# iamarkaj/AwesomeSLAM

Hardware: AMD Instinct MI355X
Metric: EKF/UKF filter-steps/s @ N_landmarks (higher is better)
Workload: dtype f32

## Files before the change

awesomeslam_amd/csrc/aslam_core.hip:

```cpp
#include "../../include/aslam_core.h"
#include "../../include/aslam_scan.h"

#include <hip/hip_runtime.h>

#include <cmath>
#include <cstdio>
#include <cstring>
#include <cstdlib>
#include <algorithm>
#include <mutex>
#include <string>
#include <type_traits>
#include <vector>

#include "ekf_small.h"
#include "ekf_large.h"
#include "ekf_large_launch.h"
#include "scan_front.h"
#if ASLAM_HAVE_UKF
#include "ukf_small.h"
#include "ukf_large.h"
#include "ukf_large_launch.h"
#endif

// ... 103 lines not shown
template <typename F> int with_large_view(aslam_ctx *c, F &&f)
{
        return c->cfg.dtype == ASLAM_F32 ? f(c->lv32) : f(c->lv64);
}

int seed_pose_block(double *P, size_t B, size_t NP)
{
        std::vector<double> blk(3 * NP, 0.0);
        for (int i = 0; i < 3; ++i)
                blk[(size_t)i * NP + i] = (double)KP_ROBOT_POSE;
        for (size_t b = 0; b < B; ++b)
                HIP_TRY(hipMemcpy(P + b * NP * NP, blk.data(), sizeof(double) * blk.size(), hipMemcpyHostToDevice));
        return ASLAM_OK;
}

template <typename T> int init_P_large(aslam_ctx *c, LargeView<T> &lv)
{
        const size_t B = c->cfg.batch, NP = c->NP;
        HIP_TRY(hipMemset(lv.P, 0, sizeof(double) * B * NP * NP));
        HIP_TRY(hipMemset(lv.G, 0, sizeof(T) * B * NP * NP));
        HIP_TRY(hipMemset(lv.S, 0, sizeof(T) * B * NP * NP));
        if (lv.Vw)
                HIP_TRY(hipMemset(lv.Vw, 0, sizeof(T) * B * NP * NP));
        return seed_pose_block(lv.P, B, NP);
}

int init_state(aslam_ctx *c)
{
        const int B = c->cfg.batch, NP = c->NP;
        DevView &d = c->dv;
        HIP_TRY(hipMemset(d.X, 0, sizeof(double) * B * NP));
        HIP_TRY(hipMemset(d.Z, 0, sizeof(double) * B * NP));
        if (!c->large)
                HIP_TRY(hipMemset(d.P, 0, sizeof(double) * (size_t)B * NP * NP));
        HIP_TRY(hipMemset(d.status, 0, sizeof(uint32_t) * B));
        HIP_TRY(hipMemset(d.sens_n, 0, sizeof(int) * B));
        HIP_TRY(hipMemset(d.wait_n, 0, sizeof(int) * B));
        std::vector<int> n(B, 3), fl(B, FLAG_INIT_X | FLAG_INIT_Z);
        std::vector<double> A(2 * (size_t)B, 0.0);
        for (int b = 0; b < B; ++b)
                A[2 * b] = 1.0;
        HIP_TRY(hipMemcpy(d.n, n.data(), sizeof(int) * B, hipMemcpyHostToDevice));
        HIP_TRY(hipMemcpy(d.flags, fl.data(), sizeof(int) * B, hipMemcpyHostToDevice));
        HIP_TRY(hipMemcpy(d.A, A.data(), sizeof(double) * 2 * B, hipMemcpyHostToDevice));
        if (c->large)
                return with_large_view(c, [&](auto &lv) { return init_P_large(c, lv); });
// ... 80 lines not shown

template <typename T> int alloc_large(aslam_ctx *c, LargeView<T> &lv)
{
        const size_t B = (size_t)c->cfg.batch, NP = (size_t)c->NP;
        const LargePlan plan = large_plan(sizeof(T) == 4, c->NP, c->cfg.batch, c->cfg.batch, c->lh.knobs);
        int rc = ASLAM_OK;
        auto A_ = [&](int r) {
                if (rc == ASLAM_OK)
                        rc = r;
        };
        lv.NP = c->NP;
        lv.xrows = c->cfg.filter == ASLAM_UKF ? 2 : 1;
        A_(dev_alloc(c, &lv.P, B * NP * NP, c->owned));
        c->largeP = lv.P;
        A_(dev_alloc(c, &lv.G, B * NP * NP, c->owned));
        A_(dev_alloc(c, &lv.S, B * NP * NP, c->owned));
        A_(dev_alloc(c, &lv.Hc, B * (NP / 2) * 4, c->owned));
        A_(dev_alloc(c, &lv.Y, B * NP, c->owned));
        A_(dev_alloc(c, &lv.Linv, B * LARGE_NB_MAX * LB * LB, c->owned));
        if (plan.need_Lpl)
                A_(dev_alloc(c, &lv.Lpl, B * LPlanes::per_filter((int)NP), c->owned));
        if (plan.need_Vw)
                A_(dev_alloc(c, &lv.Vw, B * NP * NP, c->owned));
        return rc;
}

#if ASLAM_HAVE_UKF
int ukf_large_alloc(aslam_ctx *c)
{
        const size_t B = (size_t)c->cfg.batch, NP = (size_t)c->NP;
        const size_t MP = 2 * NP + 16;
        UkfLargeView &u = c->ukfl;
        u.MP = (int)MP;
        int rc = dev_alloc(c, &u.D, B * NP * MP, c->owned);
        if (rc == ASLAM_OK)
                rc = dev_alloc(c, &u.DZ, B * NP * MP, c->owned);
        if (rc == ASLAM_OK)
                rc = dev_alloc(c, &u.XP, B * 3 * MP, c->owned);
        if (rc == ASLAM_OK)
                rc = dev_alloc(c, &u.Xbar, B * NP, c->owned);
        if (rc == ASLAM_OK)
                rc = dev_alloc(c, &u.sc, B * 8, c->owned);
        return rc;
}
#endif
}
// ... 691 lines not shown
                *stream_groups = c->large ? c->lh.last_groups : 0;
        if (chol_resident)
                *chol_resident = c->large && c->lh.last_plan.chain == LargeChain::F32_RESIDENT;
        if (launches_per_callback)
                *launches_per_callback = c->large ? c->lh.last_plan.launches : 1;
        return ASLAM_OK;
}

int aslam_kernel_info(aslam_ctx *c, char *name, int name_cap, int *grid, int *block, int *lds_bytes)
{
        if (!c)
                return fail(ASLAM_ERR_ARG, "null context");
        char buf[192];
        size_t lds = 0;
        if (c->large)
        {
                const LargePlan plan = large_plan(c->cfg.dtype == ASLAM_F32, c->NP, c->cfg.batch, c->cfg.batch, c->lh.knobs);
#if ASLAM_HAVE_UKF
                if (c->cfg.filter == ASLAM_UKF)
                        std::snprintf(buf, sizeof(buf), "ukf_large_wabt + large_update_panel<double> + large_syrk<double> (%d-launch chain per callback, 1 stream)",
                                      ukf_large_plan(c->NP).launches);
                else
#endif
                if (plan.chain == LargeChain::F32_RESIDENT)
                        std::snprintf(buf, sizeof(buf), "%s + %s + large_syrk_bf16x3 (%d-launch chain per callback, %d stream groups)",
                                      plan.chol16 ? "large_chol_bf16" : "large_chol_resident", plan.trsm16 ? "large_trsm_bf16" : "large_trsm_pipe<17>",
                                      plan.launches, c->lh.knobs.groups);
                else if (plan.chain == LargeChain::F32_RIGHT)
                        std::snprintf(buf, sizeof(buf), "large_right_step + large_syrk_bf16x3 (%d-launch chain per callback: one right-looking launch per block column)", plan.launches);
                else if (plan.chain == LargeChain::F32_LEFT)
                        std::snprintf(buf, sizeof(buf), "large_trsm_pipe<17> + large_syrk_bf16x3 (%d-launch chain per callback: multi-workgroup Cholesky)", plan.launches);
                else
                        std::snprintf(buf, sizeof(buf), "large_update_panel<double> (%d-launch chain per callback, %d stream groups)", plan.launches, c->lh.knobs.groups);
                lds = LargeLds::bytes(c->NP);
        }
        else if (c->cfg.filter == ASLAM_EKF)
        {
                std::snprintf(buf, sizeof(buf), "ekf_small_kernel<%d,0>", c->NT);
                lds = with_NT(c->NT, [](auto nt) -> size_t { return SmallLayout<decltype(nt)::value>::total; });
        }
#if ASLAM_HAVE_UKF
        else
        {
                std::snprintf(buf, sizeof(buf), "ukf_small_kernel<%d,0>", c->NT);
                lds = with_NT(c->NT, [](auto nt) -> size_t { return UkfLayout<decltype(nt)::value>::total; });
        }
#endif
// ... 16 lines not shown
```

awesomeslam_amd/csrc/ekf_large.h:

```cpp
#pragma once

#include <type_traits>

#include "small_common.h"

namespace aslam
{
constexpr int LB = 64;
constexpr int LARGE_OBS_CAP = 1024;
constexpr int LARGE_WAIT_CAP = 2048;
constexpr int LARGE_NP_MAX = 1088;
constexpr int LARGE_NB_MAX = LARGE_NP_MAX / LB;

template <typename T> struct LargeView
{
        int NP;
        double *P;
        T *G;
        T *S;
        double *Hc;
        double *Y;
        T *Linv;
        T *Vw;
        unsigned short *Lpl;
        int xrows;
};

typedef float f4 __attribute__((ext_vector_type(4)));
template <typename T> struct Mfma;
template <> struct Mfma<double>
{
        typedef d4 acc_t;
        static __device__ __forceinline__ acc_t zero()
        {
                return (acc_t){0.0, 0.0, 0.0, 0.0};
        }
        static __device__ __forceinline__ acc_t mma(double a, double b, acc_t c)
        {
                return __builtin_amdgcn_mfma_f64_16x16x4f64(a, b, c, 0, 0, 0);
        }
        static __device__ __forceinline__ int row(int lane, int r)
        {
                return (lane >> 4) + 4 * r;
        }
};
template <> struct Mfma<float>
{
        typedef f4 acc_t;
// ... 25 lines not shown
                const bf2 mm = __builtin_convertvector(r1, bf2);
                const f2 r2 = r1 - __builtin_convertvector(mm, f2);
                const bf2 ll = __builtin_convertvector(r2, bf2);
                h[e] = __builtin_bit_cast(unsigned, hh), m[e] = __builtin_bit_cast(unsigned, mm), l[e] = __builtin_bit_cast(unsigned, ll);
        }
}

struct LPlanes
{
        unsigned short *base;
        __host__ __device__ static size_t per_filter(int NP) { return (size_t)3 * NP * NP; }
        __host__ __device__ unsigned short *Lq(int b, int NP) const { return base + (size_t)b * per_filter(NP); }
        __host__ __device__ unsigned short *block(int b, int NP, int k, int j) const { return Lq(b, NP) + (size_t)(64 * k) * NP + 64 * j; }
};
__host__ __device__ __forceinline__ int lplane_pos(int c)
{
        return 32 * (c >> 5) + 8 * ((c >> 2) & 3) + 4 * ((c >> 4) & 1) + (c & 3);
}

__host__ __device__ __forceinline__ int large_blocks(int n, int xrows = 1)
{
        return (n + xrows + LB - 1) / LB;
}

struct LargeLds
{
        static __host__ __device__ size_t bytes(int NP)
        {
                size_t o = 0;
                o += 8 * (size_t)NP * 2;
                o += 4 * (size_t)LARGE_OBS_CAP * 6;
                o += 4 * (size_t)LARGE_WAIT_CAP * 5;
                o += 4 * (size_t)(NP / 2);
                o += 4 * (size_t)LARGE_OBS_CAP * 4 * 2;
                o += 4 * (size_t)NP;
                o = (o + 15) & ~(size_t)15;
                return o + sizeof(SmallShared);
        }
        static __device__ __forceinline__ SmallLds carve(unsigned char *smem, int NP)
        {
                SmallLds L;
                unsigned char *p = smem;
                L.Lt = nullptr;
                L.Dinv = nullptr;
                L.sY = nullptr;
                L.sU = nullptr;
// ... 810 lines not shown
                        }
                }
}

#ifndef ASLAM_XU_ROWS
#define ASLAM_XU_ROWS 8
#endif
constexpr int XU_ROWS = ASLAM_XU_ROWS;
template <int DIAG = 0, int PL = 0>
__global__ __launch_bounds__(256, 3) void large_syrk_bf16x3(DevView d, LargeView<float> lv, LPlanes vpl, int nfilters, const int *skipped)
{
        constexpr int TB = 128, KC = 32;
        constexpr int LDB = KC;
        typedef __bf16 bf8 __attribute__((ext_vector_type(8)));
        typedef unsigned u4 __attribute__((ext_vector_type(4)));
        typedef unsigned u2 __attribute__((ext_vector_type(2)));
        __shared__ __attribute__((aligned(16))) unsigned short As[3][TB * LDB];
        __shared__ __attribute__((aligned(16))) unsigned short Bs[3][TB * LDB];
        const int ntile = (lv.NP + TB - 1) / TB, nlow = ntile * (ntile + 1) / 2;
        const int slot = blockIdx.x >> 3;
        const int b = (slot / nlow) * 8 + (blockIdx.x & 7);
        if (b >= nfilters || skipped[b])
                return;
        const int n = d.n[b], NP = lv.NP;
        const int na = large_blocks(n) * LB;
        const int tl = slot % nlow;
        int rt = (int)((sqrtf(8.0f * (float)tl + 1.0f) - 1.0f) * 0.5f);
        while ((rt + 1) * (rt + 2) / 2 <= tl)
                ++rt;
        while (rt * (rt + 1) / 2 > tl)
                --rt;
        const int jt = tl - rt * (rt + 1) / 2;
        if (rt * TB >= n)
                return;
        const int tid = threadIdx.x, wave = tid >> 6, lane = tid & 63, li = lane & 15, lg = lane >> 4;
        const int wr = (wave >> 1) * 64, wc = (wave & 1) * 64;
        const float *G = lv.G + (size_t)b * NP * NP;
        double *P = lv.P + (size_t)b * NP * NP;
        constexpr int LPR = KC / 4, RPP = 256 / LPR, NPASS = TB / RPP;
        const int lrow = tid / LPR, lc0 = (tid % LPR) * 4;
        const float *Ap[NPASS], *Bp[NPASS];
#pragma unroll
        for (int q = 0; q < NPASS; ++q)
        {
                Ap[q] = G + (size_t)min(rt * TB + lrow + RPP * q, na - 1) * NP + lc0;
                Bp[q] = G + (size_t)min(jt * TB + lrow + RPP * q, na - 1) * NP + lc0;
        }
        f4 acc[4][4];
#pragma unroll
        for (int u = 0; u < 4; ++u)
#pragma unroll
                for (int v = 0; v < 4; ++v)
                        acc[u][v] = (f4){0.f, 0.f, 0.f, 0.f};
        f4 ta[NPASS], tb[NPASS];
        auto fetch = [&](int kc) {
                if constexpr (PL)
                        return;
#pragma unroll
                for (int q = 0; q < NPASS; ++q)
                {
                        ta[q] = *reinterpret_cast<const f4 *>(Ap[q] + kc);
                        tb[q] = *reinterpret_cast<const f4 *>(Bp[q] + kc);
                }
        };
        typedef __attribute__((address_space(3))) unsigned short lds_us;
        const __amdgpu_buffer_rsrc_t vrs = __builtin_amdgcn_make_buffer_rsrc(PL ? (void *)vpl.Lq(b, NP) : (void *)nullptr, 0, (int)(LPlanes::per_filter(NP) * 2), 0x00020000);
        const unsigned dma_vo = (unsigned)(((lane >> 2) * NP) * 2 + (((lane & 3) ^ (lane >> 4)) * 16));
        const unsigned ldsA = (unsigned)__builtin_amdgcn_readfirstlane((int)((unsigned)(uintptr_t)(lds_us *)&As[0][0] + (unsigned)wave * 2048u));
        const unsigned ldsB = (unsigned)__builtin_amdgcn_readfirstlane((int)((unsigned)(uintptr_t)(lds_us *)&Bs[0][0] + (unsigned)wave * 2048u));
        auto dma_slab = [&](int kc) {
                const unsigned plane_b = (unsigned)(NP * NP * 2);
                const unsigned soA = (unsigned)__builtin_amdgcn_readfirstlane(((rt * TB + 32 * wave) * NP + kc) * 2);
                const unsigned soB = (unsigned)__builtin_amdgcn_readfirstlane(((jt * TB + 32 * wave) * NP + kc) * 2);
                const unsigned r16 = (unsigned)(16 * NP * 2);
#pragma unroll
                for (int p = 0; p < 3; ++p)
#pragma unroll
                        for (int jj = 0; jj < 2; ++jj)
                        {
                                asm volatile("s_add_u32 m0, %0, %1\n\ts_nop 0\n\tbuffer_load_dwordx4 %2, %3, %4 offen lds"
                                             :
                                             : "s"(ldsA), "n"(p * TB * LDB * 2 + jj * 1024), "v"(dma_vo), "s"(vrs), "s"(soA + (unsigned)p * plane_b + (unsigned)jj * r16)
                                             : "m0", "scc", "memory");
                                asm volatile("s_add_u32 m0, %0, %1\n\ts_nop 0\n\tbuffer_load_dwordx4 %2, %3, %4 offen lds"
                                             :
// ... 5 lines not shown
        typedef __bf16 bf2 __attribute__((ext_vector_type(2)));
        auto stash = [&](unsigned short (&S)[3][TB * LDB], int off, const f4 &x) {
                unsigned pk[3][2];
#pragma unroll
                for (int e = 0; e < 2; ++e)
                {
                        const f2 v = {x[2 * e], x[2 * e + 1]};
                        const bf2 h = __builtin_convertvector(v, bf2);
                        const f2 r1 = v - __builtin_convertvector(h, f2);
                        const bf2 m = __builtin_convertvector(r1, bf2);
                        const f2 r2 = r1 - __builtin_convertvector(m, f2);
                        const bf2 l = __builtin_convertvector(r2, bf2);
                        pk[0][e] = __builtin_bit_cast(unsigned, h), pk[1][e] = __builtin_bit_cast(unsigned, m), pk[2][e] = __builtin_bit_cast(unsigned, l);
                }
#pragma unroll
                for (int p = 0; p < 3; ++p)
                        *reinterpret_cast<u2 *>(&S[p][off]) = (u2){pk[p][0], pk[p][1]};
        };
        const bool idle = (rt == jt && wc > wr);
        const bool diagq = (rt == jt && wc == wr);
        const int nu = idle ? 0 : __builtin_amdgcn_readfirstlane(max(0, min(4, (n - (rt * TB + wr) + 15) >> 4)));
        const int nv = idle ? 0 : __builtin_amdgcn_readfirstlane(max(0, min(4, (n - (jt * TB + wc) + 15) >> 4)));
        const bool full = !(DIAG & 2) && nu == 4 && nv == 4 && !diagq;
        const int kend = min(na, (n + KC - 1) / KC * KC);
        const int a_off = (wr + li) * LDB + 8 * (lg ^ (li >> 2)), b_off = (wc + li) * LDB + 8 * (lg ^ (li >> 2));
        const int s_off = lrow * LDB + 8 * ((lc0 >> 3) ^ ((lrow & 15) >> 2)) + (lc0 & 4);
        fetch(0);
        for (int kc = 0; kc < kend; kc += KC)
        {
                if constexpr (PL)
                {
                        dma_slab(kc);
                        asm volatile("s_waitcnt vmcnt(0)" ::: "memory");
                }
                else if (!(DIAG & 4) || kc == 0)
                {
#pragma unroll
                        for (int q = 0; q < NPASS; ++q)
                        {
                                stash(As, s_off + RPP * q * LDB, ta[q]);
                                stash(Bs, s_off + RPP * q * LDB, tb[q]);
                        }
                }
                else
                {
#pragma unroll
                        for (int q = 0; q < NPASS; ++q)
                                asm volatile("" ::"v"(ta[q]), "v"(tb[q]));
                }
                if (!(DIAG & 32))
                        __syncthreads();
                if (kc + KC < kend)
                        fetch(kc + KC);
#define ASLAM_MM(t, bb, aa, c) t = __builtin_amdgcn_mfma_f32_16x16x32_bf16(__builtin_bit_cast(bf8, bb), __builtin_bit_cast(bf8, aa), c, 0, 0, 0)
                if (DIAG & 8)
                {
                }
                else if (full)
                {
#pragma unroll
                        for (int vh = 0; vh < 4; vh += 2)
                        {
                                u4 bq[2][3];
#pragma unroll
                                for (int v = 0; v < 2; ++v)
#pragma unroll
                                        for (int p = 0; p < 3; ++p)
                                        {
                                                if (DIAG & 16)
                                                        asm volatile("" : "=v"(bq[v][p]));
                                                else
                                                        bq[v][p] = *reinterpret_cast<const u4 *>(&Bs[p][b_off + 16 * (vh + v) * LDB]);
                                        }
                                f4 pa = {0.f, 0.f, 0.f, 0.f}, pb = {0.f, 0.f, 0.f, 0.f};
// ... 211 lines not shown
        {
                for (int j = VW * lane; j < n; j += 64 * VW)
                {
                        const vec_t v = *reinterpret_cast<const vec_t *>(vrow + j), w = *reinterpret_cast<const vec_t *>(q + j);
#pragma unroll
                        for (int e = 0; e < VW; ++e)
                                acc = fma((double)v[e], (double)w[e], acc);
                }
        }
        acc = wave_sum_dpp(acc);
        if (lane == 63)
        {
                const double xa = d.X[(size_t)b * NP + a] + acc;
                d.X[(size_t)b * NP + a] = xa;
                if (MODE == MODE_REPLAY)
                {
                        if (a < 3 && poses_out)
                                poses_out[((size_t)b * nsteps + s) * 3 + a] = xa;
                        if (a == 0 && dims_out)
                                dims_out[(size_t)b * nsteps + s] = n;
                }
        }
}
template <int MODE>
__device__ __forceinline__ void x_update_rows_body(float (*sh)[LARGE_NP_MAX], const DevView &d, const LargeView<float> &lv, int b, int xb, int n, int s, int nsteps,
                                                   double *poses_out, int32_t *dims_out)
{
        const int NP = lv.NP;
        const int tid = threadIdx.x, lane = tid & 63;
        if (xb * 4 * XU_ROWS >= n)
                return;
        const float *G = lv.G + (size_t)b * NP * NP;
        for (int j = 4 * tid; j < NP; j += 4 * 256)
        {
                *reinterpret_cast<f4 *>(&sh[0][j]) = *reinterpret_cast<const f4 *>(G + (size_t)n * NP + j);
                *reinterpret_cast<f4 *>(&sh[1][j]) = *reinterpret_cast<const f4 *>(G + j);
                *reinterpret_cast<f4 *>(&sh[2][j]) = *reinterpret_cast<const f4 *>(G + NP + j);
                *reinterpret_cast<f4 *>(&sh[3][j]) = *reinterpret_cast<const f4 *>(G + 2 * (size_t)NP + j);
        }
        __syncthreads();
        double *P = lv.P + (size_t)b * NP * NP;
        const int a0 = (xb * 4 + (tid >> 6)) * XU_ROWS;
        constexpr int NPASS = 5;
        auto load_row = [&](f4 (&v)[NPASS], int a) {
                const float *vr = G + (size_t)min(a, n - 1) * NP;
#pragma unroll
                for (int i = 0; i < NPASS; ++i)
// ... 50 lines not shown
                        prow[a] -= dd;
                        const double xa = d.X[(size_t)b * NP + a] + acc;
                        d.X[(size_t)b * NP + a] = xa;
                        if (MODE == MODE_REPLAY)
                        {
                                if (a < 3 && poses_out)
                                        poses_out[((size_t)b * nsteps + s) * 3 + a] = xa;
                                if (a == 0 && dims_out)
                                        dims_out[(size_t)b * nsteps + s] = n;
                        }
                }
        }
}

template <int MODE>
__global__ __launch_bounds__(256) void large_x_update_rows(DevView d, LargeView<float> lv, int s, int nsteps, double *poses_out, int32_t *dims_out, const int *skipped)
{
        __shared__ __attribute__((aligned(16))) float sh[4][LARGE_NP_MAX];
        const int b = blockIdx.y;
        if (skipped[b])
                return;
        x_update_rows_body<MODE>(sh, d, lv, b, (int)blockIdx.x, d.n[b], s, nsteps, poses_out, dims_out);
}
}

#include "ekf_large_trsm.h"
#include "ekf_large_chol.h"
#include "ekf_large_trsm16.h"
```

awesomeslam_amd/csrc/ekf_large_launch.h:

```cpp
#pragma once

#include <hip/hip_runtime.h>

#include <algorithm>
#include <cstdlib>

#include "ekf_large.h"
#include "aslam_large16.h"

namespace aslam
{
constexpr int LARGE_GROUPS_MAX = 8;
constexpr int CHOL_RESIDENT_MIN_BATCH = 32;

struct LargeKnobs
{
        int groups = 3;
        int chol_resident = -1;
        int right_step = 1;
        int bf16_pipe = 3;
        int keep_l32 = 0;
        int gs_tiles = 0;
        int syrk_running = 0;
};

inline LargeKnobs large_knobs_from_env()
{
        LargeKnobs k;
        auto flag = [](const char *name, int &v) { if (const char *e = std::getenv(name)) v = std::atoi(e) != 0; };
        if (const char *e = std::getenv("ASLAM_LARGE_GROUPS"))
                k.groups = std::max(1, std::min(LARGE_GROUPS_MAX, std::atoi(e)));
        if (const char *e = std::getenv("ASLAM_BF16_PIPE"))
                k.bf16_pipe = std::atoi(e) & 3;
        flag("ASLAM_CHOL_RESIDENT", k.chol_resident);
        flag("ASLAM_RIGHT_STEP", k.right_step);
        flag("ASLAM_KEEP_L32", k.keep_l32);
        flag("ASLAM_GS_TILES", k.gs_tiles);
        flag("ASLAM_SYRK_RUNNING", k.syrk_running);
        return k;
}

enum class LargeChain
{
        F64_LEFT,
        F32_RESIDENT,
        F32_RIGHT,
        F32_LEFT
};

struct LargePlan
{
        LargeChain chain;
        bool chol16, trsm16;
        bool chol_f32out;
        bool gs_tiles, syrk_running;
        int launches;
        bool need_Lpl, need_Vw;
};

inline LargePlan large_plan(bool f32, int NP, int batch, int filters, const LargeKnobs &k)
{
        const int NB = NP / LB;
        auto resident = [&k](int nf) { return k.chol_resident >= 0 ? k.chol_resident != 0 : nf >= CHOL_RESIDENT_MIN_BATCH; };
        LargePlan p = {};
        p.gs_tiles = k.gs_tiles != 0;
        p.syrk_running = k.syrk_running != 0;
        p.need_Lpl = f32 && k.bf16_pipe != 0;
        p.need_Vw = f32 && k.right_step && !resident(batch);
        if (!f32)
                p.chain = LargeChain::F64_LEFT, p.launches = 4 + 2 * NB;
        else if (resident(filters))
        {
                p.chain = LargeChain::F32_RESIDENT, p.launches = 6;
                p.chol16 = (k.bf16_pipe & 2) != 0;
                p.trsm16 = (k.bf16_pipe & 1) != 0;
                p.chol_f32out = !p.trsm16 || k.keep_l32;
        }
        else if (p.need_Vw)
                p.chain = LargeChain::F32_RIGHT, p.launches = 5 + NB;
        else
                p.chain = LargeChain::F32_LEFT, p.launches = 4 + 2 * NB;
        return p;
}

struct LargeHost
{
        LargeKnobs knobs;
        hipStream_t aux[LARGE_GROUPS_MAX - 1] = {};
        hipEvent_t ev_fork = nullptr, ev_join[LARGE_GROUPS_MAX - 1] = {};
        int last_groups = 0;
        LargePlan last_plan = {};
};

inline DevView shifted(DevView d, size_t b, bool trace)
{
        const size_t np = (size_t)d.NP, T_ = (size_t)d.T;
        d.X += b * np;
        d.Z += b * np;
        d.A += 2 * b;
// ... 11 lines not shown
                d.tr_pose += 2 * b * T_;
                d.tr_yaw += b * T_;
                d.tr_twist += 2 * b * T_;
                d.tr_dt += b * T_;
                d.tr_new += b * T_;
                d.tr_nobs += b * T_;
                d.tr_obs += b * T_ * (size_t)d.max_obs * 2;
        }
        return d;
}

template <typename T> LargeView<T> shifted(LargeView<T> v, size_t b)
{
        const size_t np = (size_t)v.NP;
        v.P += b * np * np;
        v.G += b * np * np;
        v.S += b * np * np;
        v.Hc += b * (np / 2) * 4;
        v.Linv += b * LARGE_NB_MAX * LB * LB;
        if (v.Lpl)
                v.Lpl += b * LPlanes::per_filter((int)np);
        if (v.Vw)
                v.Vw += b * np * np;
        v.Y += b * np;
        return v;
}

template <typename T> struct LargeGroup
{
        DevView dv;
        LargeView<T> v;
        int *skip;
        double *poses;
        int32_t *dims;
        int nb;
        hipStream_t st;
};

template <typename T, int MODE>
void launch_large_chain(const LargePlan &plan, const LargeGroup<T> &g, size_t lds, int64_t t0, int s, int nsteps, StepArgs sa)
{
        const int NP = g.v.NP, NB = NP / LB, gb = g.nb;
        hipLaunchKernelGGL((large_frontend_kernel<T, MODE>), dim3(gb), dim3(SMALL_WG), lds, g.st, g.dv, g.v, t0 + s, s, nsteps, g.poses, g.dims, sa, g.skip);
        if (plan.gs_tiles)
                hipLaunchKernelGGL(large_build_GS_tiles<T>, dim3(NB * (NB + 1) / 2, gb), dim3(256), 0, g.st, g.dv, g.v, g.skip);
        else
                hipLaunchKernelGGL(large_build_GS<T>, dim3(1 + (NP / 2 + GS_ROW_PAIRS - 1) / GS_ROW_PAIRS, gb), dim3(256), 0, g.st, g.dv, g.v, g.skip);
        const int ntile = (NP + 127) / 128;
        const dim3 syrk_grid(8 * (ntile * (ntile + 1) / 2) * ((gb + 7) / 8));
        if constexpr (sizeof(T) == 8)
        {
                for (int k = 0; k < NB; ++k)
                {
                        hipLaunchKernelGGL(large_potrf_inv_tiles<T>, dim3(gb), dim3(256), 0, g.st, g.dv, g.v, k, g.skip);
                        hipLaunchKernelGGL(large_update_panel<T>, dim3((2 * NB - k) / 2, 1, gb), dim3(256), 0, g.st, g.dv, g.v, k, 0, g.skip);
                }
                hipLaunchKernelGGL(large_syrk<T>, syrk_grid, dim3(256), 0, g.st, g.dv, g.v, gb, g.skip);
                hipLaunchKernelGGL((large_x_update<T, MODE, false>), dim3((NP + 3) / 4, gb), dim3(256), 0, g.st, g.dv, g.v, s, nsteps, g.poses, g.dims, g.skip);
        }
        else
        {
                LargeView<T> vv = g.v;
                switch (plan.chain)
                {
                case LargeChain::F32_RESIDENT:
                        if (plan.chol16)
                                launch_chol_bf16(g.dv, g.v, gb, g.skip, g.st, plan.chol_f32out);
                        else
                                hipLaunchKernelGGL(large_chol_resident<LARGE_NB_MAX>, dim3(gb), dim3(256), 0, g.st, g.dv, g.v, g.skip);
                        if (plan.trsm16)
                                launch_trsm_bf16(g.dv, g.v, gb, g.skip, g.st);
                        else
                                hipLaunchKernelGGL(large_trsm_pipe<LARGE_NB_MAX>, dim3(8 * ((gb + 7) / 8) * NB), dim3(256), 0, g.st, g.dv, g.v, gb, g.skip);
                        break;
                case LargeChain::F32_RIGHT:
                        hipLaunchKernelGGL(large_potrf_inv_tiles<T>, dim3(gb), dim3(256), 0, g.st, g.dv, g.v, 0, g.skip);
                        for (int k = 0; k < NB; ++k)
                        {
                                const int M = NB - k - 1;
                                hipLaunchKernelGGL(large_right_step<0>, dim3(M * (M + 1) / 2 + NB * M + NB, 1, gb), dim3(256), 0, g.st, g.dv, g.v, k, g.skip);
                        }
                        vv.G = g.v.Vw;
                        break;
                default:
                        for (int k = 0; k < NB; ++k)
                        {
                                hipLaunchKernelGGL(large_potrf_inv_tiles<T>, dim3(gb), dim3(256), 0, g.st, g.dv, g.v, k, g.skip);
                                if (k + 1 < NB)
                                        hipLaunchKernelGGL(large_update_panel<T>, dim3((NB - k) / 2, 1, gb), dim3(256), 0, g.st, g.dv, g.v, k, 1, g.skip);
                        }
                        hipLaunchKernelGGL(large_trsm_pipe<LARGE_NB_MAX>, dim3(8 * ((gb + 7) / 8) * NB), dim3(256), 0, g.st, g.dv, g.v, gb, g.skip);
                }
                if (plan.syrk_running)
                        hipLaunchKernelGGL((large_syrk_bf16x3<2>), syrk_grid, dim3(256), 0, g.st, g.dv, vv, LPlanes{nullptr}, gb, g.skip);
                else
                        hipLaunchKernelGGL((large_syrk_bf16x3<0>), syrk_grid, dim3(256), 0, g.st, g.dv, vv, LPlanes{nullptr}, gb, g.skip);
                hipLaunchKernelGGL((large_x_update_rows<MODE>), dim3((NP + 4 * XU_ROWS - 1) / (4 * XU_ROWS), gb), dim3(256), 0, g.st, g.dv, vv, s, nsteps, g.poses,
                                   g.dims, g.skip);
        }
}

template <int MODE, typename T>
hipError_t launch_large(LargeHost &h, const DevView &dv, const LargeView<T> &lv, int *skipped, int64_t t0, int nsteps, double *poses, int32_t *dims,
                        StepArgs sa, hipStream_t st)
{
        const size_t lds = LargeLds::bytes(dv.NP);
        if (hipError_t e = hipFuncSetAttribute(reinterpret_cast<const void *>(large_frontend_kernel<T, MODE>), hipFuncAttributeMaxDynamicSharedMemorySize, (int)lds))
                return e;
        const bool one = MODE == MODE_STEP && sa.traj >= 0;
        const int first = one ? sa.traj : 0, Bz = one ? 1 : dv.B;
        sa.traj = one ? 0 : sa.traj;
        const LargePlan plan = large_plan(sizeof(T) == 4, dv.NP, dv.B, Bz, h.knobs);
        const bool split = Bz >= std::max(32, 8 * h.knobs.groups);
        const int NG = split ? h.knobs.groups : 1;
        const int per = split ? ((Bz + NG - 1) / NG + 7) & ~7 : Bz;
        LargeGroup<T> g[LARGE_GROUPS_MAX];
        h.last_plan = plan;
        h.last_groups = 0;
        for (int q = 0; q < NG; ++q)
        {
                const int o = std::min(q * per, Bz);
                const size_t b0 = (size_t)(first + o);
                g[q] = {shifted(dv, b0, MODE == MODE_REPLAY), shifted(lv, b0), skipped + b0, poses, dims, std::min(per, Bz - o), q == 0 ? st : h.aux[q - 1]};
                if (MODE == MODE_REPLAY && poses)
                        g[q].poses += b0 * (size_t)nsteps * 3;
                if (MODE == MODE_REPLAY && dims)
                        g[q].dims += b0 * (size_t)nsteps;
                h.last_groups += g[q].nb > 0;
        }
        hipError_t e = split ? hipEventRecord(h.ev_fork, st) : hipSuccess;
        for (int q = 1; q < NG && e == hipSuccess; ++q)
// ... 14 lines not shown
```

awesomeslam_amd/csrc/ekf_large_trsm16.h:

```cpp
#pragma once

namespace aslam
{
namespace t16
{
typedef unsigned u4v __attribute__((ext_vector_type(4)));
typedef unsigned u2v __attribute__((ext_vector_type(2)));
typedef __bf16 bf8 __attribute__((ext_vector_type(8)));
typedef __bf16 bf2 __attribute__((ext_vector_type(2)));
typedef float f2v __attribute__((ext_vector_type(2)));

constexpr int PLD = LB;
constexpr int PLANE = LB * PLD;
constexpr int BLK = 3 * PLANE;
constexpr int NBUF = 5;

typedef LPlanes Planes;
__host__ __device__ __forceinline__ int perm_pos(int c)
{
        return lplane_pos(c);
}

__device__ __forceinline__ void split2(float a, float b, unsigned &h, unsigned &m, unsigned &l)
{
// ... 413 lines not shown
        }
        (void)nb_rows;
}
}

template <int NBMAX, int STAMP = 0>
__global__ __launch_bounds__(256, 1) void large_trsm_bf16(DevView d, LargeView<float> lv, t16::Planes pl, int nfilters, const int *skipped)
{
        using namespace t16;
        static_assert(NBMAX == 17, "the chain lists 17 block columns");
        __shared__ __attribute__((aligned(1024))) unsigned short lds[NBUF][BLK];
        __shared__ __attribute__((aligned(1024))) float gl[4][16 * LB];
        const int NP = lv.NP, nblk = NP / LB;
        const int slot = blockIdx.x >> 3;
        const int b = (slot / nblk) * 8 + (blockIdx.x & 7), rb = slot % nblk;
        if (b >= nfilters || skipped[b])
                return;
        const int n = d.n[b];
        const int nb = large_blocks(n);
        if (rb >= nb)
                return;
        const int tid = threadIdx.x, wave = tid >> 6, lane = tid & 63, li = lane & 15, lg = lane >> 4;
        const int wv = __builtin_amdgcn_readfirstlane(wave);
        Rows rows;
        rows.rsrc = __builtin_amdgcn_make_buffer_rsrc(uniform_ptr(lv.G + (size_t)b * NP * NP), 0, NP * NP * 4, 0x00020000);
        rows.so0 = (unsigned)((LB * rb + 16 * wv) * NP * 4);
        rows.out = lv.G + (size_t)b * NP * NP + (size_t)(LB * rb + 16 * wave + li) * NP + 4 * lg;
        rows.rq = rows.rsrc, rows.vq = 0, rows.qplane = 0;
        asm volatile("" ::: "a0", "a255");
        Pipe pp;
        Regs R;
        f4 c[4];
        asm volatile("; ASLAM_STRIP_LIVE_BEGIN vmem: global_store_dwordx4=4" ::: "memory");
        sweep16<STAMP, false>(c, R, pp, lds, gl[wv], pl, b, nb, nb, NP, rows, tid);
        asm volatile("; ASLAM_STRIP_LIVE_END" ::: "memory");
        if constexpr (STAMP)
                if (tid == 0 && blockIdx.x == 0)
                        for (int i = 0; i < 13; ++i)
                                lv.Y[i] = (double)pp.ph[i];
}

template <int NBMAX, bool F32OUT = true>
__global__ __launch_bounds__(256, 1) void large_chol_bf16(DevView d, LargeView<float> lv, t16::Planes pl, const int *skipped)
{
        using namespace t16;
        static_assert(NBMAX == 17, "the chain lists 17 block columns");
        constexpr int PIPE_BYTES = NBUF * BLK * 2, TILE_BYTES = chol64::TILES * TSZ * (int)sizeof(double);
        static_assert(TILE_BYTES <= PIPE_BYTES, "the tiles of the diagonal factorisation alias the block buffers");
        __shared__ __attribute__((aligned(1024))) unsigned short lds[NBUF][BLK];
        __shared__ __attribute__((aligned(1024))) float gl[4][16 * LB];
        double *tiles = reinterpret_cast<double *>(&lds[0][0]);
        const int b = blockIdx.x;
        if (skipped[b])
                return;
        const int n = d.n[b], NP = lv.NP;
        const int nb = large_blocks(n);
        const int tid0 = threadIdx.x;
        const int wv = __builtin_amdgcn_readfirstlane(tid0 >> 6);
        float *Sb = lv.S + (size_t)b * NP * NP;
        float *Linv = lv.Linv + (size_t)b * LARGE_NB_MAX * LB * LB;
        asm volatile("" ::: "a0", "a255");
        Rows rows;
        rows.rsrc = __builtin_amdgcn_make_buffer_rsrc(uniform_ptr(Sb), 0, NP * NP * 4, 0x00020000);
        rows.rq = __builtin_amdgcn_make_buffer_rsrc(uniform_ptr(pl.Lq(b, NP)), 0, 3 * NP * NP * 2, 0x00020000);
        rows.qplane = (unsigned)(NP * NP * 2);
        bool ok = true;
        Pipe pp;
        Regs R;
#pragma unroll 1
        for (int I = 0; I < nb; ++I)
        {
                int tid = tid0;
                asm volatile("" : "+v"(tid));
                const int wave = tid >> 6, lane = tid & 63, li = lane & 15, lg = lane >> 4;
                rows.so0 = (unsigned)((LB * I + 16 * wv) * NP * 4);
                rows.out = Sb + (size_t)(LB * I + 16 * wave + li) * NP + 4 * lg;
                rows.vq = (unsigned)(((LB * I + 16 * wave + li) * NP + 8 * lg) * 2);
                f4 c[4];
                if constexpr (F32OUT)
// ... 66 lines not shown
```

Baseline: 37680.

## Add bordered Cholesky path when landmark count barely spills into a new block

Result: faster. 38660 (median of 6 runs) (+2.6%).

```diff
diff --git a/awesomeslam_amd/csrc/aslam_core.hip b/awesomeslam_amd/csrc/aslam_core.hip
--- a/awesomeslam_amd/csrc/aslam_core.hip
+++ b/awesomeslam_amd/csrc/aslam_core.hip
@@ -149,6 +149,8 @@
         HIP_TRY(hipMemset(lv.S, 0, sizeof(T) * B * NP * NP));
         if (lv.Vw)
                 HIP_TRY(hipMemset(lv.Vw, 0, sizeof(T) * B * NP * NP));
+        if (lv.V2)
+                HIP_TRY(hipMemset(lv.V2, 0, sizeof(float) * B * NP * 4));
         return seed_pose_block(lv.P, B, NP);
 }
 
@@ -275,6 +277,8 @@
                 A_(dev_alloc(c, &lv.Lpl, B * LPlanes::per_filter((int)NP), c->owned));
         if (plan.need_Vw)
                 A_(dev_alloc(c, &lv.Vw, B * NP * NP, c->owned));
+        if (plan.need_V2)
+                A_(dev_alloc(c, &lv.V2, B * NP * 4, c->owned));
         return rc;
 }
 
@@ -1012,7 +1016,10 @@
                                       ukf_large_plan(c->NP).launches);
                 else
 #endif
-                if (plan.chain == LargeChain::F32_RESIDENT)
+                if (plan.chain == LargeChain::F32_RESIDENT && plan.border)
+                        std::snprintf(buf, sizeof(buf), "large_chol_bf16 + large_trsm_bf16 + large_syrk_bf16x3, bordered (n mod 64 <= 3: %d-launch chain per callback, %d stream groups)",
+                                      plan.launches, c->lh.knobs.groups);
+                else if (plan.chain == LargeChain::F32_RESIDENT)
                         std::snprintf(buf, sizeof(buf), "%s + %s + large_syrk_bf16x3 (%d-launch chain per callback, %d stream groups)",
                                       plan.chol16 ? "large_chol_bf16" : "large_chol_resident", plan.trsm16 ? "large_trsm_bf16" : "large_trsm_pipe<17>",
                                       plan.launches, c->lh.knobs.groups);
diff --git a/awesomeslam_amd/csrc/ekf_large.h b/awesomeslam_amd/csrc/ekf_large.h
--- a/awesomeslam_amd/csrc/ekf_large.h
+++ b/awesomeslam_amd/csrc/ekf_large.h
@@ -24,6 +24,8 @@
         T *Vw;
         unsigned short *Lpl;
         int xrows;
+        float *V2;
+        int border;
 };
 
 typedef float f4 __attribute__((ext_vector_type(4)));
@@ -95,6 +97,18 @@
 {
         return (n + xrows + LB - 1) / LB;
 }
+
+struct LargeBorder
+{
+        int nbf, r;
+        bool bordered;
+};
+__host__ __device__ __forceinline__ LargeBorder large_border(int n, bool enabled = true)
+{
+        const int nbf = n / LB, r = n - LB * nbf;
+        return {nbf, r, enabled && nbf >= 1 && r >= 1 && r <= 3};
+}
+constexpr int BORDER_MAX = 3;
 
 struct LargeLds
 {
@@ -951,8 +965,11 @@
         const int b = (slot / nlow) * 8 + (blockIdx.x & 7);
         if (b >= nfilters || skipped[b])
                 return;
-        const int n = d.n[b], NP = lv.NP;
-        const int na = large_blocks(n) * LB;
+        const int NP = lv.NP;
+        const int na = large_blocks(d.n[b]) * LB;
+        const LargeBorder lb = large_border(d.n[b], lv.border != 0);
+        const int R0 = LB * lb.nbf;
+        const int n = lb.bordered ? R0 : d.n[b];
         const int tl = slot % nlow;
         int rt = (int)((sqrtf(8.0f * (float)tl + 1.0f) - 1.0f) * 0.5f);
         while ((rt + 1) * (rt + 2) / 2 <= tl)
@@ -990,6 +1007,15 @@
                 {
                         ta[q] = *reinterpret_cast<const f4 *>(Ap[q] + kc);
                         tb[q] = *reinterpret_cast<const f4 *>(Bp[q] + kc);
+                }
+        };
+        auto point_at_border = [&](int kc) {
+                const float *V2 = lv.V2 + (size_t)b * NP * 4 - kc;
+#pragma unroll
+                for (int q = 0; q < NPASS; ++q)
+                {
+                        Ap[q] = V2 + 4 * (lc0 ? na - 1 : min(rt * TB + lrow + RPP * q, na - 1));
+                        Bp[q] = V2 + 4 * (lc0 ? na - 1 : min(jt * TB + lrow + RPP * q, na - 1));
                 }
         };
         typedef __attribute__((address_space(3))) unsigned short lds_us;
@@ -1041,7 +1067,8 @@
         const int nu = idle ? 0 : __builtin_amdgcn_readfirstlane(max(0, min(4, (n - (rt * TB + wr) + 15) >> 4)));
         const int nv = idle ? 0 : __builtin_amdgcn_readfirstlane(max(0, min(4, (n - (jt * TB + wc) + 15) >> 4)));
         const bool full = !(DIAG & 2) && nu == 4 && nv == 4 && !diagq;
-        const int kend = min(na, (n + KC - 1) / KC * KC);
+        const bool bslab = !PL && lb.bordered;
+        const int kend = bslab ? R0 + KC : min(na, (n + KC - 1) / KC * KC);
         const int a_off = (wr + li) * LDB + 8 * (lg ^ (li >> 2)), b_off = (wc + li) * LDB + 8 * (lg ^ (li >> 2));
         const int s_off = lrow * LDB + 8 * ((lc0 >> 3) ^ ((lrow & 15) >> 2)) + (lc0 & 4);
         fetch(0);
@@ -1069,6 +1096,8 @@
                 }
                 if (!(DIAG & 32))
                         __syncthreads();
+                if (bslab && kc + KC == R0)
+                        point_at_border(R0);
                 if (kc + KC < kend)
                         fetch(kc + KC);
 #define ASLAM_MM(t, bb, aa, c) t = __builtin_amdgcn_mfma_f32_16x16x32_bf16(__builtin_bit_cast(bf8, bb), __builtin_bit_cast(bf8, aa), c, 0, 0, 0)
@@ -1326,7 +1355,7 @@
                 }
         }
 }
-template <int MODE>
+template <int MODE, int XU_ROWS = aslam::XU_ROWS>
 __device__ __forceinline__ void x_update_rows_body(float (*sh)[LARGE_NP_MAX], const DevView &d, const LargeView<float> &lv, int b, int xb, int n, int s, int nsteps,
                                                    double *poses_out, int32_t *dims_out)
 {
@@ -1423,6 +1452,259 @@
                 return;
         x_update_rows_body<MODE>(sh, d, lv, b, (int)blockIdx.x, d.n[b], s, nsteps, poses_out, dims_out);
 }
+struct BorderLds
+{
+        static constexpr int NROW = 4 + 2 * BORDER_MAX;
+        static constexpr int R0MAX = (LARGE_NP_MAX / LB - 1) * LB;
+        static constexpr int NDOT = (BORDER_MAX * (BORDER_MAX + 1)) / 2 + (4 + BORDER_MAX) * BORDER_MAX;
+        static constexpr int ROW_BYTES = NROW * R0MAX * 4;
+        static constexpr int BYTES = ROW_BYTES + 8 * (NDOT + BORDER_MAX * BORDER_MAX + BORDER_MAX + (4 + BORDER_MAX) * BORDER_MAX);
+        static_assert(ROW_BYTES >= 4 * LARGE_NP_MAX * 4, "the unbordered body's rows");
+};
+
+template <int MODE, int XU_ROWS = 8>
+__global__ __launch_bounds__(256) void large_x_update_border(DevView d, LargeView<float> lv, int s, int nsteps, double *poses_out, int32_t *dims_out, const int *skipped)
+{
+        extern __shared__ __attribute__((aligned(16))) unsigned char xu_smem[];
+        const int b = blockIdx.y;
+        if (skipped[b])
+                return;
+        const int n = d.n[b], NP = lv.NP;
+        const LargeBorder lb = large_border(n, lv.border != 0);
+        if (!lb.bordered)
+        {
+                x_update_rows_body<MODE, XU_ROWS>(reinterpret_cast<float(*)[LARGE_NP_MAX]>(xu_smem), d, lv, b, (int)blockIdx.x, n, s, nsteps, poses_out, dims_out);
+                return;
+        }
+        constexpr int RM = BORDER_MAX, R0MAX = BorderLds::R0MAX;
+        const int xb = blockIdx.x;
+        if (xb * 4 * XU_ROWS >= n)
+                return;
+        const int R0 = LB * lb.nbf, r = lb.r;
+        float(*sh)[R0MAX] = reinterpret_cast<float(*)[R0MAX]>(xu_smem);
+        double *dots = reinterpret_cast<double *>(xu_smem + BorderLds::ROW_BYTES);
+        double *sL = dots + BorderLds::NDOT;
+        double *sinv = sL + RM * RM;
+        double *sV2 = sinv + RM;
+        const int tid = threadIdx.x, lane = tid & 63, wave = tid >> 6;
+        const float *G = lv.G + (size_t)b * NP * NP;
+        const float *S = lv.S + (size_t)b * NP * NP;
+        if (tid < BorderLds::NDOT)
+        {
+                double raw;
+                if (tid < 6)
+                {
+                        const int s_ = tid < 1 ? 0 : tid < 3 ? 1 : 2, t_ = tid - s_ * (s_ + 1) / 2;
+                        raw = (s_ < r && t_ < r) ? (double)S[(size_t)(R0 + s_) * NP + R0 + t_] : (s_ == t_ ? 1.0 : 0.0);
+                }
+                else
+                {
+                        const int w = (tid - 6) / RM, t_ = (tid - 6) % RM;
+                        const int vrow = w == 0 ? n : w < 4 ? w - 1 : R0 + (w - 4);
+                        raw = (t_ < r && w - 4 < r) ? (double)G[(size_t)vrow * NP + R0 + t_] : 0.0;
+                }
+                dots[tid] = raw;
+        }
+        for (int j = 4 * tid; j < R0; j += 4 * 256)
+        {
+                const f4 z = {0.f, 0.f, 0.f, 0.f};
+                *reinterpret_cast<f4 *>(&sh[0][j]) = *reinterpret_cast<const f4 *>(G + (size_t)n * NP + j);
+                *reinterpret_cast<f4 *>(&sh[1][j]) = *reinterpret_cast<const f4 *>(G + j);
+                *reinterpret_cast<f4 *>(&sh[2][j]) = *reinterpret_cast<const f4 *>(G + NP + j);
+                *reinterpret_cast<f4 *>(&sh[3][j]) = *reinterpret_cast<const f4 *>(G + 2 * (size_t)NP + j);
+#pragma unroll
+                for (int t = 0; t < RM; ++t)
+                {
+                        *reinterpret_cast<f4 *>(&sh[4 + t][j]) = t < r ? *reinterpret_cast<const f4 *>(S + (size_t)(R0 + t) * NP + j) : z;
+                        *reinterpret_cast<f4 *>(&sh[7 + t][j]) = t < r ? *reinterpret_cast<const f4 *>(G + (size_t)(R0 + t) * NP + j) : z;
+                }
+        }
+        __syncthreads();
+        for (int p = wave; p < BorderLds::NDOT; p += 4)
+        {
+                int ra, rb;
+                if (p < 6)
+                {
+                        const int s_ = p < 1 ? 0 : p < 3 ? 1 : 2, t_ = p - s_ * (s_ + 1) / 2;
+                        ra = 4 + s_, rb = 4 + t_;
+                }
+                else
+                {
+                        const int w = (p - 6) / RM, t_ = (p - 6) % RM;
+                        ra = w < 4 ? w : 7 + (w - 4), rb = 4 + t_;
+                }
+                double acc = 0.0;
+                for (int j = 4 * lane; j < R0; j += 256)
+                {
+                        const f4 x = *reinterpret_cast<const f4 *>(&sh[ra][j]), y = *reinterpret_cast<const f4 *>(&sh[rb][j]);
+#pragma unroll
+                        for (int e = 0; e < 4; ++e)
+                                acc = fma((double)x[e], (double)y[e], acc);
+                }
+                acc = wave_sum_dpp(acc);
+                if (lane == 63)
+                        dots[p] -= acc;
+        }
+        __syncthreads();
+        if (tid == 0)
+        {
+                double L[RM][RM], inv[RM];
+                bool ok = true;
+                for (int s_ = 0; s_ < RM; ++s_)
+                        for (int t_ = 0; t_ <= s_; ++t_)
+                        {
+                                double m = dots[s_ * (s_ + 1) / 2 + t_];
+                                for (int u = 0; u < t_; ++u)
+                                        m -= L[s_][u] * L[t_][u];
+                                if (s_ == t_)
+                                {
+                                        ok = ok && (m > 0.0);
+                                        L[s_][s_] = sqrt(m);
+                                        inv[s_] = 1.0 / L[s_][s_];
+                                }
+                                else
+                                        L[s_][t_] = m * inv[t_];
+                        }
+                for (int s_ = 0; s_ < RM; ++s_)
+                {
+                        for (int t_ = 0; t_ <= s_; ++t_)
+                                sL[s_ * RM + t_] = L[s_][t_];
+                        sinv[s_] = inv[s_];
+                }
+                for (int w = 0; w < 4 + RM; ++w)
+                {
+                        double v2[RM];
+                        for (int t_ = 0; t_ < RM; ++t_)
+                        {
+                                double c = dots[6 + RM * w + t_];
+                                for (int u = 0; u < t_; ++u)
+                                        c -= v2[u] * L[t_][u];
+                                c *= inv[t_];
+                                v2[t_] = c;
+                                sV2[w * RM + t_] = c;
+                        }
+                }
+                if (!ok && xb == 0)
+                        atomicOr(&d.status[b], 4u);
+        }
+        __syncthreads();
+        double *P = lv.P + (size_t)b * NP * NP;
+        float *V2g = lv.V2 + (size_t)b * NP * 4;
+        if (xb == 0 && tid == 0)
+                *reinterpret_cast<f4 *>(V2g + 4 * (size_t)(large_blocks(n) * LB - 1)) = (f4){0.f, 0.f, 0.f, 0.f};
+        const int a0 = (xb * 4 + wave) * XU_ROWS;
+        constexpr int NPASS = R0MAX / 256;
+        auto load_row = [&](f4 (&v)[NPASS], f4 &vb, int a) {
+                const float *vr = G + (size_t)min(a, n - 1) * NP;
+#pragma unroll
+                for (int i = 0; i < NPASS; ++i)
+                {
+                        const int j = 4 * lane + 256 * i;
+                        v[i] = j < R0 ? *reinterpret_cast<const f4 *>(vr + j) : (f4){0.f, 0.f, 0.f, 0.f};
+                }
+                vb = *reinterpret_cast<const f4 *>(vr + R0);
+        };
+        f4 vn[NPASS], vbn;
+        load_row(vn, vbn, a0);
+#pragma unroll 1
+        for (int rr = 0; rr < XU_ROWS; ++rr)
+        {
+                const int a = a0 + rr;
+                if (a >= n)
+                        break;
+                f4 v[NPASS];
+                const f4 vb = vbn;
+#pragma unroll
+                for (int i = 0; i < NPASS; ++i)
+                        v[i] = vn[i];
+                if (rr + 1 < XU_ROWS)
+                        load_row(vn, vbn, a + 1);
+                double acc = 0.0, dd = 0.0, dp[3] = {0.0, 0.0, 0.0}, el[RM] = {0.0, 0.0, 0.0}, ft[RM] = {0.0, 0.0, 0.0};
+#pragma unroll
+                for (int i = 0; i < NPASS; ++i)
+                {
+                        const int j = 4 * lane + 256 * i;
+                        if (j >= R0)
+                                continue;
+                        f4 o[BorderLds::NROW];
+#pragma unroll
+                        for (int w = 0; w < BorderLds::NROW; ++w)
+                                o[w] = *reinterpret_cast<const f4 *>(&sh[w][j]);
+#pragma unroll
+                        for (int e = 0; e < 4; ++e)
+                        {
+                                const double ve = (double)v[i][e];
+                                acc = fma(ve, (double)o[0][e], acc);
+                                dd = fma(ve, ve, dd);
+#pragma unroll
+                                for (int t = 0; t < 3; ++t)
+                                {
+                                        dp[t] = fma(ve, (double)o[1 + t][e], dp[t]);
+                                        el[t] = fma(ve, (double)o[4 + t][e], el[t]);
+                                        ft[t] = fma(ve, (double)o[7 + t][e], ft[t]);
+                                }
+                        }
+                }
+                acc = wave_sum_dpp(acc), dd = wave_sum_dpp(dd);
+#pragma unroll
+                for (int t = 0; t < 3; ++t)
+                        dp[t] = wave_sum_dpp(dp[t]), el[t] = wave_sum_dpp(el[t]), ft[t] = wave_sum_dpp(ft[t]);
+                if (lane == 63)
+                {
+                        double v2[RM];
+#pragma unroll
+                        for (int t = 0; t < RM; ++t)
+                        {
+                                double c = 0.0;
+                                if (t < r)
+                                {
+                                        c = (double)vb[t] - el[t];
+                                        for (int u = 0; u < t; ++u)
+                                                c -= v2[u] * sL[t * RM + u];
+                                        c *= sinv[t];
+                                }
+                                v2[t] = c;
+                        }
+                        *reinterpret_cast<f4 *>(V2g + 4 * (size_t)a) = (f4){(float)v2[0], (float)v2[1], (float)v2[2], 0.f};
+                        double *prow = P + (size_t)a * NP;
+#pragma unroll
+                        for (int t = 0; t < RM; ++t)
+                        {
+                                acc = fma(v2[t], sV2[t], acc);
+                                dd = fma(v2[t], v2[t], dd);
+#pragma unroll
+                                for (int j = 0; j < 3; ++j)
+                                        dp[j] = fma(v2[t], sV2[(1 + j) * RM + t], dp[j]);
+                        }
+                        for (int j = 0; j < 3 && j < a; ++j)
+                        {
+                                const double pn = prow[j] - dp[j];
+                                prow[j] = pn;
+                                P[(size_t)j * NP + a] = pn;
+                        }
+                        prow[a] -= dd;
+                        for (int t = 0; t < r; ++t)
+                                if (a >= 3 && (a < R0 || R0 + t < a))
+                                {
+                                        double bt = ft[t];
+                                        for (int u = 0; u < RM; ++u)
+                                                bt = fma(v2[u], sV2[(4 + t) * RM + u], bt);
+                                        const double pn = prow[R0 + t] - bt;
+                                        prow[R0 + t] = pn;
+                                        P[(size_t)(R0 + t) * NP + a] = pn;
+                                }
+                        const double xa = d.X[(size_t)b * NP + a] + acc;
+                        d.X[(size_t)b * NP + a] = xa;
+                        if (MODE == MODE_REPLAY)
+                        {
+                                if (a < 3 && poses_out)
+                                        poses_out[((size_t)b * nsteps + s) * 3 + a] = xa;
+                                if (a == 0 && dims_out)
+                                        dims_out[(size_t)b * nsteps + s] = n;
+                        }
+                }
+        }
+}
 }
 
 #include "ekf_large_trsm.h"
diff --git a/awesomeslam_amd/csrc/ekf_large_launch.h b/awesomeslam_amd/csrc/ekf_large_launch.h
--- a/awesomeslam_amd/csrc/ekf_large_launch.h
+++ b/awesomeslam_amd/csrc/ekf_large_launch.h
@@ -21,6 +21,8 @@
         int bf16_pipe = 3;
         int keep_l32 = 0;
         int gs_tiles = 0;
+        int border = 1;
+        int border_rows = 8;
         int syrk_running = 0;
 };
 
@@ -37,6 +39,9 @@
         flag("ASLAM_KEEP_L32", k.keep_l32);
         flag("ASLAM_GS_TILES", k.gs_tiles);
         flag("ASLAM_SYRK_RUNNING", k.syrk_running);
+        flag("ASLAM_BORDER", k.border);
+        if (const char *e = std::getenv("ASLAM_BORDER_ROWS"))
+                k.border_rows = std::atoi(e) >= 32 ? 32 : std::atoi(e) >= 16 ? 16 : 8;
         return k;
 }
 
@@ -52,10 +57,12 @@
 {
         LargeChain chain;
         bool chol16, trsm16;
+        int border_rows;
+        bool border;
         bool chol_f32out;
         bool gs_tiles, syrk_running;
         int launches;
-        bool need_Lpl, need_Vw;
+        bool need_Lpl, need_Vw, need_V2;
 };
 
 inline LargePlan large_plan(bool f32, int NP, int batch, int filters, const LargeKnobs &k)
@@ -67,6 +74,7 @@
         p.syrk_running = k.syrk_running != 0;
         p.need_Lpl = f32 && k.bf16_pipe != 0;
         p.need_Vw = f32 && k.right_step && !resident(batch);
+        p.need_V2 = f32 && k.border && k.bf16_pipe == 3 && !k.keep_l32;
         if (!f32)
                 p.chain = LargeChain::F64_LEFT, p.launches = 4 + 2 * NB;
         else if (resident(filters))
@@ -75,6 +83,8 @@
                 p.chol16 = (k.bf16_pipe & 2) != 0;
                 p.trsm16 = (k.bf16_pipe & 1) != 0;
                 p.chol_f32out = !p.trsm16 || k.keep_l32;
+                p.border_rows = k.border_rows;
+                p.border = k.border != 0 && p.chol16 && p.trsm16 && !k.keep_l32;
         }
         else if (p.need_Vw)
                 p.chain = LargeChain::F32_RIGHT, p.launches = 5 + NB;
@@ -132,6 +142,8 @@
                 v.Lpl += b * LPlanes::per_filter((int)np);
         if (v.Vw)
                 v.Vw += b * np * np;
+        if (v.V2)
+                v.V2 += b * np * 4;
         v.Y += b * np;
         return v;
 }
@@ -171,17 +183,33 @@
         else
         {
                 LargeView<T> vv = g.v;
+                vv.border = plan.border;
+                const dim3 xu_grid((NP + 4 * XU_ROWS - 1) / (4 * XU_ROWS), gb);
                 switch (plan.chain)
                 {
                 case LargeChain::F32_RESIDENT:
                         if (plan.chol16)
-                                launch_chol_bf16(g.dv, g.v, gb, g.skip, g.st, plan.chol_f32out);
+                                launch_chol_bf16(g.dv, vv, gb, g.skip, g.st, plan.chol_f32out);
                         else
                                 hipLaunchKernelGGL(large_chol_resident<LARGE_NB_MAX>, dim3(gb), dim3(256), 0, g.st, g.dv, g.v, g.skip);
                         if (plan.trsm16)
-                                launch_trsm_bf16(g.dv, g.v, gb, g.skip, g.st);
+                                launch_trsm_bf16(g.dv, vv, gb, g.skip, g.st);
                         else
                                 hipLaunchKernelGGL(large_trsm_pipe<LARGE_NB_MAX>, dim3(8 * ((gb + 7) / 8) * NB), dim3(256), 0, g.st, g.dv, g.v, gb, g.skip);
+                        if (plan.border)
+                        {
+                                auto xu = [&](auto rows) {
+                                        constexpr int R = decltype(rows)::value;
+                                        hipLaunchKernelGGL((large_x_update_border<MODE, R>), dim3((NP + 4 * R - 1) / (4 * R), gb), dim3(256), BorderLds::BYTES, g.st, g.dv, vv, s,
+                                                           nsteps, g.poses, g.dims, g.skip);
+                                };
+                                if (plan.border_rows == 16)
+                                        xu(std::integral_constant<int, 16>{});
+                                else if (plan.border_rows == 32)
+                                        xu(std::integral_constant<int, 32>{});
+                                else
+                                        xu(std::integral_constant<int, 8>{});
+                        }
                         break;
                 case LargeChain::F32_RIGHT:
                         hipLaunchKernelGGL(large_potrf_inv_tiles<T>, dim3(gb), dim3(256), 0, g.st, g.dv, g.v, 0, g.skip);
@@ -205,8 +233,8 @@
                         hipLaunchKernelGGL((large_syrk_bf16x3<2>), syrk_grid, dim3(256), 0, g.st, g.dv, vv, LPlanes{nullptr}, gb, g.skip);
                 else
                         hipLaunchKernelGGL((large_syrk_bf16x3<0>), syrk_grid, dim3(256), 0, g.st, g.dv, vv, LPlanes{nullptr}, gb, g.skip);
-                hipLaunchKernelGGL((large_x_update_rows<MODE>), dim3((NP + 4 * XU_ROWS - 1) / (4 * XU_ROWS), gb), dim3(256), 0, g.st, g.dv, vv, s, nsteps, g.poses,
-                                   g.dims, g.skip);
+                if (!plan.border)
+                        hipLaunchKernelGGL((large_x_update_rows<MODE>), xu_grid, dim3(256), 0, g.st, g.dv, vv, s, nsteps, g.poses, g.dims, g.skip);
         }
 }
 
@@ -217,6 +245,14 @@
         const size_t lds = LargeLds::bytes(dv.NP);
         if (hipError_t e = hipFuncSetAttribute(reinterpret_cast<const void *>(large_frontend_kernel<T, MODE>), hipFuncAttributeMaxDynamicSharedMemorySize, (int)lds))
                 return e;
+        if constexpr (sizeof(T) == 4)
+        {
+                const void *xu[3] = {reinterpret_cast<const void *>(large_x_update_border<MODE, 8>), reinterpret_cast<const void *>(large_x_update_border<MODE, 16>),
+                                     reinterpret_cast<const void *>(large_x_update_border<MODE, 32>)};
+                for (const void *f : xu)
+                        if (hipError_t e = hipFuncSetAttribute(f, hipFuncAttributeMaxDynamicSharedMemorySize, BorderLds::BYTES))
+                                return e;
+        }
         const bool one = MODE == MODE_STEP && sa.traj >= 0;
         const int first = one ? sa.traj : 0, Bz = one ? 1 : dv.B;
         sa.traj = one ? 0 : sa.traj;
diff --git a/awesomeslam_amd/csrc/ekf_large_trsm16.h b/awesomeslam_amd/csrc/ekf_large_trsm16.h
--- a/awesomeslam_amd/csrc/ekf_large_trsm16.h
+++ b/awesomeslam_amd/csrc/ekf_large_trsm16.h
@@ -459,17 +459,22 @@
                 return;
         const int tid = threadIdx.x, wave = tid >> 6, lane = tid & 63, li = lane & 15, lg = lane >> 4;
         const int wv = __builtin_amdgcn_readfirstlane(wave);
+        const LargeBorder lbd = large_border(n, lv.border != 0);
+        const int nbk = lbd.bordered ? lbd.nbf : nb;
+        const bool tail = lbd.bordered && rb == lbd.nbf, tailS = tail && wv == 0;
+        const int row0 = LB * rb + 16 * (tail ? max(wv - 1, 0) : wv);
+        float *M = (tailS ? lv.S : lv.G) + (size_t)b * NP * NP;
         Rows rows;
-        rows.rsrc = __builtin_amdgcn_make_buffer_rsrc(uniform_ptr(lv.G + (size_t)b * NP * NP), 0, NP * NP * 4, 0x00020000);
-        rows.so0 = (unsigned)((LB * rb + 16 * wv) * NP * 4);
-        rows.out = lv.G + (size_t)b * NP * NP + (size_t)(LB * rb + 16 * wave + li) * NP + 4 * lg;
+        rows.rsrc = __builtin_amdgcn_make_buffer_rsrc(uniform_ptr(M), 0, NP * NP * 4, 0x00020000);
+        rows.so0 = (unsigned)(row0 * NP * 4);
+        rows.out = M + (size_t)(row0 + li) * NP + 4 * lg;
         rows.rq = rows.rsrc, rows.vq = 0, rows.qplane = 0;
         asm volatile("" ::: "a0", "a255");
         Pipe pp;
         Regs R;
         f4 c[4];
         asm volatile("; ASLAM_STRIP_LIVE_BEGIN vmem: global_store_dwordx4=4" ::: "memory");
-        sweep16<STAMP, false>(c, R, pp, lds, gl[wv], pl, b, nb, nb, NP, rows, tid);
+        sweep16<STAMP, false>(c, R, pp, lds, gl[wv], pl, b, nbk, nb, NP, rows, tid);
         asm volatile("; ASLAM_STRIP_LIVE_END" ::: "memory");
         if constexpr (STAMP)
                 if (tid == 0 && blockIdx.x == 0)
@@ -491,7 +496,8 @@
         if (skipped[b])
                 return;
         const int n = d.n[b], NP = lv.NP;
-        const int nb = large_blocks(n);
+        const LargeBorder lbd = large_border(n, lv.border != 0);
+        const int nb = lbd.bordered ? lbd.nbf : large_blocks(n);
         const int tid0 = threadIdx.x;
         const int wv = __builtin_amdgcn_readfirstlane(tid0 >> 6);
         float *Sb = lv.S + (size_t)b * NP * NP;
```
